# Lain-Iwakuro/Plonky2-Demo

Measured on AMD Instinct MI355X. Metric: proofs/sec for m=64 matmul circuit (full prove(), PoseidonGoldilocksConfig, standard_recursion_config), higher is better.
Workload: dtype u64 (Goldilocks, 64-bit modular integer)

## Files before the change

plonky2_demo_amd/csrc/gl64_gfx950.cuh:

```cuda
#pragma once
#include "gl64.cuh"

#if defined(__HIP_DEVICE_COMPILE__)
typedef uint32_t glx_u32x2 __attribute__((ext_vector_type(2)));
__device__ __forceinline__ gl_t glx_mk64(uint32_t lo, uint32_t hi) { glx_u32x2 v = {lo, hi}; return __builtin_bit_cast(gl_t, v); }
__device__ __forceinline__ gl_t glx_add_eps_if(gl_t z, uint32_t bit) {
    gl_t r;
    asm("v_mad_u64_u32 %0, vcc, %1, -1, %2" : "=v"(r) : "v"(bit), "v"(z) : "vcc");
    return r;
}


template <bool CANON>
__device__ __forceinline__ void glx_mul3(gl_t aA, gl_t bA, gl_t aB, gl_t bB, gl_t aC, gl_t bC, gl_t& rA, gl_t& rB, gl_t& rC) {
    typedef uint32_t u32;
    gl_t p00A, midA, p11A, p00B, midB, p11B, p00C, midC, p11C;
    uint64_t cmA, cmB, cmC;
    asm("v_mad_u64_u32 %[p00A], vcc, %[a0A], %[b0A], 0\n\t"
        "v_mad_u64_u32 %[p00B], vcc, %[a0B], %[b0B], 0\n\t"
        "v_mad_u64_u32 %[p00C], vcc, %[a0C], %[b0C], 0\n\t"
        "v_mad_u64_u32 %[midA], vcc, %[a0A], %[b1A], 0\n\t"
        "v_mad_u64_u32 %[midB], vcc, %[a0B], %[b1B], 0\n\t"
        "v_mad_u64_u32 %[midC], vcc, %[a0C], %[b1C], 0\n\t"
        "v_mad_u64_u32 %[p11A], vcc, %[a1A], %[b1A], 0\n\t"
// ... 279 lines not shown
        : [zA] "=&v"(zA), [cA] "=&s"(cA), [zB] "=&v"(zB), [cB] "=&s"(cB), [zC] "=&v"(zC), [cC] "=&s"(cC), [eA] "=&v"(eA), [eB] "=&v"(eB), [eC] "=&v"(eC)
        : [tA] "v"(topA), [loA] "v"(loA), [tB] "v"(topB), [loB] "v"(loB), [tC] "v"(topC), [loC] "v"(loC));
    rA = glx_add_eps_if(zA, eA); rB = glx_add_eps_if(zB, eB); rC = glx_add_eps_if(zC, eC);
    const uint64_t nA = whA | sA, nB = whB | sB, nC = whC | sC;
    if (__builtin_expect((wlA | wlB | wlC | nA | nB | nC) != 0, 0)) {
        u32 pA, pB, pC, mA, mB, mC;
        asm("v_cndmask_b32_e64 %[pA], 0, -1, %[wlA]\n\t"
            "v_cndmask_b32_e64 %[pB], 0, -1, %[wlB]\n\t"
            "v_cndmask_b32_e64 %[pC], 0, -1, %[wlC]\n\t"
            "v_cndmask_b32_e64 %[mA], 0, 1, %[nA]\n\t"
            "v_cndmask_b32_e64 %[mB], 0, 1, %[nB]\n\t"
            "v_cndmask_b32_e64 %[mC], 0, 1, %[nC]"
            : [pA] "=&v"(pA), [pB] "=&v"(pB), [pC] "=&v"(pC), [mA] "=&v"(mA), [mB] "=&v"(mB), [mC] "=&v"(mC)
            : [wlA] "s"(wlA), [wlB] "s"(wlB), [wlC] "s"(wlC), [nA] "s"(nA), [nB] "s"(nB), [nC] "s"(nC));
        rA = gl_sub(gl_add(rA, (gl_t)pA), (gl_t)mA); rB = gl_sub(gl_add(rB, (gl_t)pB), (gl_t)mB); rC = gl_sub(gl_add(rC, (gl_t)pC), (gl_t)mC);
    }
}

__device__ __forceinline__ gl_t glx_canon(gl_t x) { return glx_add_eps_if(x, (x >= GL_P) ? 1u : 0u); }
__device__ __forceinline__ gl_t glx_add_cc(gl_t a, gl_t b) {
    const gl_t s = a + b;
    return glx_add_eps_if(s, ((s < a) | (s >= GL_P)) ? 1u : 0u);
}
__device__ __forceinline__ gl_t glx_sub_cc(gl_t a, gl_t b) {
#ifdef GLX_C_BUTTERFLY
    const gl_t d = a - b;
    return d - ((a < b) ? GL_EPS : 0);
#endif
    uint32_t r0, r1, e;
    asm("v_sub_co_u32 %[r0], vcc, %[a0], %[b0]\n\t"
        "s_nop 1\n\t"
        "v_subb_co_u32 %[r1], vcc, %[a1], %[b1], vcc\n\t"
        "s_nop 1\n\t"
        "v_cndmask_b32_e64 %[e], 0, -1, vcc\n\t"
        "v_sub_co_u32 %[r0], vcc, %[r0], %[e]\n\t"
        "s_nop 1\n\t"
        "v_subbrev_co_u32 %[r1], vcc, 0, %[r1], vcc"
        : [r0] "=&v"(r0), [r1] "=&v"(r1), [e] "=&v"(e)
        : [a0] "v"((uint32_t)a), [a1] "v"((uint32_t)(a >> 32)), [b0] "v"((uint32_t)b), [b1] "v"((uint32_t)(b >> 32))
        : "vcc");
    return glx_mk64(r0, r1);
}
__device__ __forceinline__ void glx_sub_cc4(const gl_t (&a)[4], const gl_t (&b)[4], gl_t (&r)[4]) {
    typedef uint32_t u32;
    u32 r0A, r1A, r0B, r1B, r0C, r1C, r0D, r1D, eA, eB, eC, eD;
    uint64_t sB, sC, sD;
// ... 127 lines not shown
            : [t0] "v"((u32)term), [t1] "v"((u32)(term >> 32)),
              [wA0] "s"((u32)wA), [wA1] "s"((u32)(wA >> 32)), [wB0] "s"((u32)wB), [wB1] "s"((u32)(wB >> 32))
            : "vcc");
    }
    __device__ __forceinline__ gl_t sum(int b) const {
        gl_t r = glx_add_cc(glx_canon(a0[b]), glx_shl_c<32>(glx_canon(a1[b])));
        r = glx_add_cc(r, glx_shl_c<64>(glx_canon(a2[b])));
        r = glx_add_cc(r, glx_shl_c<64>((gl_t)k0[b]));
        r = glx_sub_cc(r, (gl_t)k1[b]);
        return glx_sub_cc(r, glx_shl_c<32>((gl_t)k2[b]));
    }
};
#elif defined(__HIPCC__)
template <bool CANON>
__device__ void glx_mul3(gl_t aA, gl_t bA, gl_t aB, gl_t bB, gl_t aC, gl_t bC, gl_t& rA, gl_t& rB, gl_t& rC);
template <bool CANON>
__device__ gl_t glx_mul(gl_t a, gl_t b);
__device__ gl_t glx_reduce96(gl_t lo, uint32_t top);
__device__ gl_t glx_mad_k(uint32_t x, uint32_t c, uint64_t k);
__device__ gl_t glx_mac_c(gl_t acc, uint32_t x, uint32_t c);
__device__ gl_t glx_canon(gl_t x);
__device__ gl_t glx_add_eps_if(gl_t z, uint32_t bit);
__device__ gl_t glx_add_cc(gl_t a, gl_t b);
__device__ gl_t glx_sub_cc(gl_t a, gl_t b);
__device__ void glx_sub_cc4(const gl_t (&a)[4], const gl_t (&b)[4], gl_t (&r)[4]);
template <int E>
__device__ gl_t glx_shl_c(gl_t x);
__device__ gl_t glx_acc_reduce(gl_t al, gl_t ah);
__device__ void glx_acc_reduce3(gl_t alA, gl_t ahA, gl_t alB, gl_t ahB, gl_t alC, gl_t ahC, gl_t& rA, gl_t& rB, gl_t& rC);
__device__ gl_t glx_mac_co(gl_t acc, uint32_t x, uint32_t c, uint64_t& carry);
__device__ void glx_acc_reduce3w(gl_t alA, gl_t ahA, uint64_t wlA, uint64_t whA, gl_t alB, gl_t ahB, uint64_t wlB, uint64_t whB,
                                 gl_t alC, gl_t ahC, uint64_t wlC, uint64_t whC, gl_t& rA, gl_t& rB, gl_t& rC);
struct GlxWideAcc2 {
    gl_t a0[2], a1[2], a2[2];
    uint32_t k0[2], k1[2], k2[2];
    __device__ void clear();
    __device__ void mac(gl_t term, gl_t wA, gl_t wB);
    __device__ gl_t sum(int b) const;
};
#endif
```

plonky2_demo_amd/csrc/merkle.hip:

```cpp
#include "context.hpp"
#include "poseidon.cuh"
#include "keccak.cuh"
#include "host_circuit.hpp"
#include <cstring>
#include <memory>

struct gl_merkle {
    gl_ctx* ctx = nullptr;
    GlMerkle tree;
    gl_t* leaves = nullptr;
    size_t num_leaves = 0, leaf_len = 0;
};

#define GL_COOP_MAX_NODES_DEFAULT 8192u
#define GL_COOP_MAX_NODES_THROUGHPUT 1024u
static uint32_t gl_coop_max_nodes() {
    static const long env = [] { const char* e = getenv("GL_COOP_MAX_NODES"); return e ? (long)strtoul(e, nullptr, 10) : -1L; }();
    if (env >= 0) return (uint32_t)env;
    return gl_proofs_in_flight.load(std::memory_order_relaxed) > 2 ? GL_COOP_MAX_NODES_THROUGHPUT : GL_COOP_MAX_NODES_DEFAULT;
}

__device__ __forceinline__ uint32_t d_bitrev(uint32_t x, uint32_t bits) { return bits ? (__brev(x) >> (32 - bits)) : 0; }

template <int WPE>
__global__ __launch_bounds__(256, WPE) void k_merkle_leaves(const gl_t* __restrict__ base, const uint64_t* __restrict__ offsets,
                                                       uint32_t leaf_len, uint32_t lg_leaves, gl_t* __restrict__ digests) {
    const uint32_t n = 1u << lg_leaves, gid = blockIdx.x * blockDim.x + threadIdx.x, r = gid < n ? gid : n - 1;
    gl_t s[12];
#pragma unroll
    for (int i = 0; i < 12; i++) s[i] = 0;
    if (leaf_len <= 4) {
        for (uint32_t e = 0; e < leaf_len; e++) s[e] = gl_canon(base[offsets[e] + r]);
    } else {
        for (uint32_t e0 = 0; e0 < leaf_len; e0 += 8) {
            const uint32_t c = leaf_len - e0 < 8 ? leaf_len - e0 : 8;
#pragma unroll
            for (int i = 0; i < 8; i++)
                if ((uint32_t)i < c) s[i] = base[offsets[e0 + i] + r];
            psd_permute_layer<PSD_LAYER_HASH>(s);
        }
    }
    if (gid >= n) return;
    const uint32_t j = d_bitrev(r, lg_leaves);
    ulonglong2* out = reinterpret_cast<ulonglong2*>(digests + 4ull * j);
    out[0] = make_ulonglong2(gl_canon(s[0]), gl_canon(s[1]));
    out[1] = make_ulonglong2(gl_canon(s[2]), gl_canon(s[3]));
}

__global__ __launch_bounds__(256, 5) void k_merkle_level(const gl_t* __restrict__ child, gl_t* __restrict__ parent, uint32_t count,
                                                         int prio ) {
    gl_raise_prio(prio);
    const uint32_t gid = blockIdx.x * blockDim.x + threadIdx.x, i = gid < count ? gid : count - 1;
    const ulonglong2* in = reinterpret_cast<const ulonglong2*>(child + 8ull * i);
    ulonglong2 a = in[0], b = in[1], c = in[2], d = in[3];
    gl_t s[12] = {a.x, a.y, b.x, b.y, c.x, c.y, d.x, d.y, 0, 0, 0, 0};
    psd_permute_layer<PSD_LAYER_HASH>(s);
    if (gid >= count) return;
    ulonglong2* out = reinterpret_cast<ulonglong2*>(parent + 4ull * i);
    out[0] = make_ulonglong2(gl_canon(s[0]), gl_canon(s[1]));
    out[1] = make_ulonglong2(gl_canon(s[2]), gl_canon(s[3]));
}

__global__ __launch_bounds__(256) void k_merkle_level_coop(const gl_t* __restrict__ child, gl_t* __restrict__ parent, uint32_t count) {
    const uint32_t gid = blockIdx.x * blockDim.x + threadIdx.x, node = gid >> 4;
    const int l = (int)(gid & 15);
    if (node >= count) return;
    gl_t s = l < 8 ? child[8ull * node + l] : 0;
    s = psd_coop_permute(s, l);
    if (l < 4) parent[4ull * node + l] = gl_canon(s);
}
__global__ __launch_bounds__(256) void k_merkle_leaves_coop(const gl_t* __restrict__ base, const uint64_t* __restrict__ offsets,
                                                            uint32_t leaf_len, uint32_t lg_leaves, gl_t* __restrict__ digests) {
    const uint32_t gid = blockIdx.x * blockDim.x + threadIdx.x, r = gid >> 4;
    const int l = (int)(gid & 15);
    if (r >= (1u << lg_leaves)) return;
    gl_t s = 0;
    if (leaf_len <= 4) {
        if ((uint32_t)l < leaf_len) s = gl_canon(base[offsets[l] + r]);
    } else {
// ... 31 lines not shown
    gl_t s[12];
#pragma unroll
    for (int k = 0; k < 12; k++) s[k] = states[12 * i + k];
    psd_permute_layer<LAYER>(s);
    if (gid >= count) return;
#pragma unroll
    for (int k = 0; k < 12; k++) states[12 * i + k] = CANON ? gl_canon(s[k]) : s[k];
}

__global__ __launch_bounds__(64, 5) void k_hash_rows(const gl_t* rows, size_t count, uint32_t len, gl_t* out) {
    const size_t gid = (size_t)blockIdx.x * blockDim.x + threadIdx.x, r = gid < count ? gid : count - 1;
    gl_t s[12];
#pragma unroll
    for (int i = 0; i < 12; i++) s[i] = 0;
    const gl_t* row = rows + r * len;
    if (len <= 4) {
        for (uint32_t e = 0; e < len; e++) s[e] = gl_canon(row[e]);
    } else {
        for (uint32_t e0 = 0; e0 < len; e0 += 8) {
            const uint32_t c = len - e0 < 8 ? len - e0 : 8;
#pragma unroll
            for (int i = 0; i < 8; i++)
                if ((uint32_t)i < c) s[i] = row[e0 + i];
            psd_permute_layer<PSD_LAYER_HASH>(s);
        }
    }
    if (gid >= count) return;
    for (int i = 0; i < 4; i++) out[4 * r + i] = gl_canon(s[i]);
}

__global__ __launch_bounds__(256) void k_kck_leaves(const gl_t* __restrict__ base, const uint64_t* __restrict__ offsets, uint32_t leaf_len,
                                                    uint32_t lg_leaves, gl_t* __restrict__ digests) {
    const uint32_t r = blockIdx.x * blockDim.x + threadIdx.x;
    if (r >= (1u << lg_leaves)) return;
    uint64_t out[4] = {0, 0, 0, 0};
    if (leaf_len * 8 <= KCK_HASH_BYTES) {
        for (uint32_t e = 0; e < leaf_len; e++) out[e] = gl_canon(base[offsets[e] + r]);
    } else {
        kck_state s;
        kck_absorb_leaf(s, leaf_len, [&](uint32_t e) { return base[offsets[e] + r]; });
        kck_digest25(s, out);
    }
    ulonglong2* o = reinterpret_cast<ulonglong2*>(digests + 4ull * d_bitrev(r, lg_leaves));
    o[0] = make_ulonglong2(out[0], out[1]);
    o[1] = make_ulonglong2(out[2], out[3]);
}
__device__ __forceinline__ void kck_node(const gl_t* __restrict__ child, gl_t* __restrict__ parent, uint32_t i) {
// ... 227 lines not shown
```

plonky2_demo_amd/csrc/poseidon.cuh:

```cuda
#pragma once
#include <stdlib.h>
#include "gl64.cuh"
#include "gl64_gfx950.cuh"
#include "poseidon_constants.h"

#if defined(__HIPCC__)
#define POSEIDON_TABLE(name, n) static __constant__ const uint64_t d_##name[n]
#define POSEIDON_TABLE32(name, n) static __constant__ const uint32_t d_##name[n]
#include "poseidon_constants.inc"
#undef POSEIDON_TABLE
#undef POSEIDON_TABLE32
#endif

#if defined(__HIP_DEVICE_COMPILE__)
#define PSD_TAB(name) d_##name
#else
#define PSD_TAB(name) name
#endif

GL_HD gl_t psd_sbox(gl_t x) {
#if defined(__HIP_DEVICE_COMPILE__)
    const gl_t x2 = glx_mul<false>(x, x), x4 = glx_mul<false>(x2, x2), x3 = glx_mul<false>(x, x2);
    return glx_mul<false>(x3, x4);
#else
// ... 76 lines not shown
        for (int i = 0; i < 12; i++) s[i] = t[i];
    }
    for (int r = 0; r < POSEIDON_PARTIAL_ROUNDS; r++) {
        const gl_t s0 = gl_add_c(psd_sbox(s[0]), POSEIDON_PARTIAL_RC[r]);
        PsdHostDot d;
        psd_host_dot_term(d, s0, 17 + 8);
        for (int i = 1; i < 12; i++) psd_host_dot_term(d, s[i], POSEIDON_PARTIAL_ROW[r * 11 + i - 1]);
        for (int i = 1; i < 12; i++) s[i] = gl_mul_add(s[i], s0, POSEIDON_PARTIAL_COL[r * 11 + i - 1]);
        s[0] = psd_host_dot_reduce(d);
    }
}

GL_HD gl_t psd_acc_reduce(gl_t al, gl_t ah) {
#if defined(__HIP_DEVICE_COMPILE__)
    return glx_acc_reduce(al, ah);
#else
    const uint32_t al_hi = (uint32_t)(al >> 32), ah_lo = (uint32_t)ah;
    const uint32_t mid = al_hi + ah_lo;
    const uint32_t top = (uint32_t)(ah >> 32) + (mid < ah_lo ? 1u : 0u);
    return gl_reduce96(((gl_t)mid << 32) | (uint32_t)al, top);
#endif
}

template <bool WITH_RC>
GL_HD void psd_mds_then_constants(gl_t (&s)[12], const gl_t* __restrict__ rc) {
    uint32_t k16 = 16, k2 = 2, k8 = 8;
#if defined(__HIP_DEVICE_COMPILE__)
    asm volatile("" : "+s"(k16), "+s"(k2), "+s"(k8));
#endif
    const uint32_t circ[12] = {17, 15, 41, k16, k2, 28, 13, 13, 39, 18, 34, 20};
    uint32_t lo[12], hi[12];
#pragma unroll
    for (int i = 0; i < 12; i++) { lo[i] = (uint32_t)s[i]; hi[i] = (uint32_t)(s[i] >> 32); }
#if defined(__HIP_DEVICE_COMPILE__)
#pragma unroll
    for (int r0 = 0; r0 < 12; r0 += 3) {
        gl_t al[3], ah[3];
#pragma unroll
        for (int k = 0; k < 3; k++) {
            const int r = r0 + k;
            if (WITH_RC) { const gl_t c = rc[r]; al[k] = glx_mad_k(lo[r], 17u, (uint64_t)(uint32_t)c); ah[k] = glx_mad_k(hi[r], 17u, c >> 32); }
            else { al[k] = (gl_t)lo[r] * 17u; ah[k] = (gl_t)hi[r] * 17u; }
#pragma unroll
            for (int i = 1; i < 12; i++) {
                al[k] += (gl_t)lo[(i + r) % 12] * circ[i];
                ah[k] += (gl_t)hi[(i + r) % 12] * circ[i];
            }
            if (r == 0) { al[k] += (gl_t)lo[0] * k8; ah[k] += (gl_t)hi[0] * k8; }
        }
        glx_acc_reduce3(al[0], ah[0], al[1], ah[1], al[2], ah[2], s[r0], s[r0 + 1], s[r0 + 2]);
    }
#else
#pragma unroll
    for (int r = 0; r < 12; r++) {
        gl_t al = 0, ah = 0;
        if (WITH_RC) { const gl_t c = rc[r]; al = (uint32_t)c; ah = c >> 32; }
#pragma unroll
        for (int i = 0; i < 12; i++) {
            al += (gl_t)lo[(i + r) % 12] * circ[i];
// ... 9 lines not shown
#define PSD_MDS_MFMA 1
#endif
#ifndef PSD_GROUP4
#define PSD_GROUP4 1
#endif
enum { PSD_LAYER_VALU = 0, PSD_LAYER_MFMA = 1, PSD_LAYER_HASH = PSD_MDS_MFMA ? PSD_LAYER_MFMA : PSD_LAYER_VALU };
#if defined(__HIPCC__)
typedef int psd_i32x4 __attribute__((ext_vector_type(4)));
typedef int psd_i32x16 __attribute__((ext_vector_type(16)));
struct PsdMfmaA { psd_i32x4 blk[4]; };
#endif
#if defined(__HIP_DEVICE_COMPILE__)
__device__ __forceinline__ PsdMfmaA psd_mfma_a() {
    const uint32_t lane = __builtin_amdgcn_mbcnt_hi(~0u, __builtin_amdgcn_mbcnt_lo(~0u, 0u)), r = lane & 31;
    const bool mine = ((r >> 2) & 1) == (lane >> 5);
    const uint32_t o8 = 8 * (r >> 3), t8 = 8 * (r & 3);
    PsdMfmaA A;
#pragma unroll
    for (int d = 0; d < 4; d++)
#pragma unroll
        for (int q = 0; q < 4; q++) A.blk[d][q] = mine ? (int)(((d_POSEIDON_MDS_I8A[4 * d + q] >> o8) & 0xFFu) << t8) : 0;
    return A;
}
__device__ __forceinline__ void psd_mds_mfma(gl_t (&s)[12], const gl_t* __restrict__ kk, const PsdMfmaA& A) {
    psd_i32x4 bl[3], bh[3];
#pragma unroll
    for (int kb = 0; kb < 3; kb++)
#pragma unroll
        for (int q = 0; q < 4; q++) {
            bl[kb][q] = (int)((uint32_t)s[4 * kb + q] ^ 0x80808080u);
            bh[kb][q] = (int)((uint32_t)(s[4 * kb + q] >> 32) ^ 0x80808080u);
        }
    int32_t one = 1, m8 = 1 << 8, m16 = 1 << 16, m24 = 1 << 24;
    asm volatile("" : "+v"(one), "+s"(m8), "+s"(m16), "+s"(m24));
    gl_t acc[2][12];
#pragma unroll
    for (int rb = 0; rb < 3; rb++) {
#pragma unroll
        for (int hf = 0; hf < 2; hf++) {
            __builtin_amdgcn_sched_barrier(0);
            psd_i32x16 d = {};
#pragma unroll
            for (int kb = 0; kb < 3; kb++)
                d = __builtin_amdgcn_mfma_i32_32x32x32_i8((rb == 0 && kb == 0) ? A.blk[3] : A.blk[(kb - rb + 3) % 3], hf ? bh[kb] : bl[kb], d, 0, 0, 0);
#pragma unroll
            for (int o = 0; o < 4; o++) {
                const int i = 4 * rb + o;
                int64_t x = (int64_t)d[4 * o] * one + (int64_t)kk[2 * i + hf];
                x += (int64_t)d[4 * o + 1] * m8;
                x += (int64_t)d[4 * o + 2] * m16;
                x += (int64_t)d[4 * o + 3] * m24;
                acc[hf][i] = (gl_t)x;
            }
        }
#pragma unroll
        for (int r0 = 3 * rb; r0 < 4 * rb + 2; r0 += 3)
            glx_acc_reduce3(acc[0][r0], acc[1][r0], acc[0][r0 + 1], acc[1][r0 + 1], acc[0][r0 + 2], acc[1][r0 + 2], s[r0], s[r0 + 1], s[r0 + 2]);
    }
    __builtin_amdgcn_sched_barrier(0);
}
#endif

GL_HD constexpr uint32_t psd_mds_entry(int r, int c) {
    constexpr uint32_t circ[12] = {17, 15, 41, 16, 2, 28, 13, 13, 39, 18, 34, 20};
    return circ[(c - r + 12) % 12] + ((r == 0 && c == 0) ? 8u : 0u);
}
GL_HD void psd_sbox_all(gl_t (&s)[12]) {
#if defined(__HIP_DEVICE_COMPILE__)
#pragma unroll
    for (int k = 0; k < 12; k += 3) {
        gl_t a2, b2, c2, a4, b4, c4, a3, b3, c3;
        glx_mul3<false>(s[k], s[k], s[k + 1], s[k + 1], s[k + 2], s[k + 2], a2, b2, c2);
        glx_mul3<false>(a2, a2, b2, b2, c2, c2, a4, b4, c4);
        glx_mul3<false>(s[k], a2, s[k + 1], b2, s[k + 2], c2, a3, b3, c3);
        glx_mul3<false>(a3, a4, b3, b4, c3, c4, s[k], s[k + 1], s[k + 2]);
    }
#else
    for (int i = 0; i < 12; i++) s[i] = psd_sbox(s[i]);
#endif
}
#if defined(__HIPCC__)
template <bool SUBST>
__device__ __forceinline__ void psd_partial_group_k(gl_t (&s)[12], const gl_t* __restrict__ K, const gl_t* in, gl_t* a) {
    uint32_t z = 0;
#if defined(__HIP_DEVICE_COMPILE__)
    asm volatile("" : "+s"(z));
#endif
    const uint32_t* __restrict__ R2 = d_POSEIDON_G3_R2 + z;
    const uint32_t* __restrict__ V1 = d_POSEIDON_G3_V1 + z;
    a[0] = s[0];
    s[0] = psd_sbox(SUBST ? in[0] : s[0]);
    uint32_t lo[12], hi[12];
#pragma unroll
// ... 63 lines not shown
    const gl_t d3 = gl_sub(psd_sbox(a3), a3);
    const uint32_t d3l = (uint32_t)d3, d3h = (uint32_t)(d3 >> 32);
    const uint32_t* __restrict__ M4 = d_POSEIDON_G4_M4 + z;
#pragma unroll
    for (int l0 = 0; l0 < 12; l0 += 3) {
        gl_t xl[3], xh[3];
        uint64_t wl[3], wh[3];
#pragma unroll
        for (int k = 0; k < 3; k++) {
            const int l = l0 + k;
            xl[k] = glx_mad_k(d3l, psd_mds_entry(l, 0), (uint64_t)(uint32_t)K[3 + l]); xh[k] = glx_mad_k(d3h, psd_mds_entry(l, 0), K[3 + l] >> 32);
#pragma unroll
            for (int i = 1; i < 12; i++) { const uint32_t c = M4[12 * l + i]; xl[k] += (gl_t)lo[i] * c; xh[k] += (gl_t)hi[i] * c; }
            { const uint32_t c = V3[l]; xl[k] += (gl_t)d1l * c; xh[k] += (gl_t)d1h * c; }
            { const uint32_t c = V2[l]; xl[k] += (gl_t)d2l * c; xh[k] += (gl_t)d2h * c; }
            { const uint32_t c = M4[12 * l]; xl[k] = glx_mac_co(xl[k], lo[0], c, wl[k]); xh[k] = glx_mac_co(xh[k], hi[0], c, wh[k]); }
        }
        glx_acc_reduce3w(xl[0], xh[0], wl[0], wh[0], xl[1], xh[1], wl[1], wh[1], xl[2], xh[2], wl[2], wh[2], s[l0], s[l0 + 1], s[l0 + 2]);
    }
}
#endif

#if defined(__HIP_DEVICE_COMPILE__)
template <int LAYER, bool WITH_RC>
__device__ __forceinline__ void psd_mds_layer(gl_t (&s)[12], int n, const PsdMfmaA& A) {
    if constexpr (LAYER == PSD_LAYER_MFMA) psd_mds_mfma(s, d_POSEIDON_MDS_K + 24 * (WITH_RC ? n : 8 + POSEIDON_PARTIAL_ROUNDS), A);
    else psd_mds_then_constants<WITH_RC>(s, WITH_RC ? d_POSEIDON_RC + 12 * n : nullptr);
}
template <int LAYER>
__device__ __forceinline__ void psd_permute_layer(gl_t (&s)[12]) {
    const gl_t* __restrict__ rc = d_POSEIDON_RC;
    PsdMfmaA A;
    if constexpr (LAYER == PSD_LAYER_MFMA) A = psd_mfma_a();
#pragma unroll
    for (int i = 0; i < 12; i++) s[i] = gl_add_c(s[i], rc[i]);
#if PSD_GROUP4
#pragma unroll 1
    for (int r = 0; r < 4; r++) { psd_sbox_all(s); if (r < 3) psd_mds_layer<LAYER, true>(s, r + 1, A); }
#pragma unroll 1
    for (int g = 0; g < POSEIDON_G4_GROUPS; g++) psd_partial_group4(s, d_POSEIDON_G4_K + 15 * g, g != 0);
    { gl_t a[3]; psd_partial_group_k<false>(s, d_POSEIDON_G4_K + 15 * POSEIDON_G4_GROUPS, nullptr, a); }
#else
#pragma unroll 1
    for (int r = 0; r < 4; r++) { psd_sbox_all(s); psd_mds_layer<LAYER, true>(s, r + 1, A); }
#pragma unroll 1
    for (int g = 0; g < POSEIDON_PARTIAL_GROUPS; g++) { gl_t a[3]; psd_partial_group<false>(s, g, nullptr, a); }
#pragma unroll 1
    for (int r = 4 + 3 * POSEIDON_PARTIAL_GROUPS; r < 4 + POSEIDON_PARTIAL_ROUNDS; r++) { s[0] = psd_sbox(s[0]); psd_mds_layer<LAYER, true>(s, r + 1, A); }
#endif
#pragma unroll 1
    for (int r = 4 + POSEIDON_PARTIAL_ROUNDS; r < 7 + POSEIDON_PARTIAL_ROUNDS; r++) { psd_sbox_all(s); psd_mds_layer<LAYER, true>(s, r + 1, A); }
    psd_sbox_all(s);
    psd_mds_layer<LAYER, false>(s, 0, A);
}
GL_HD void psd_permute(gl_t (&s)[12]) { psd_permute_layer<PSD_LAYER_VALU>(s); }
#else
#if defined(__HIPCC__)
template <int LAYER>
__device__ void psd_permute_layer(gl_t (&s)[12]);
#endif
GL_HD void psd_permute(gl_t (&s)[12]) {
    for (int r = 0; r < 4; r++) psd_full_round(s, r);
    psd_partial_rounds(s);
    for (int r = 0; r < 4; r++) psd_full_round(s, 4 + POSEIDON_PARTIAL_ROUNDS + r);
}
#endif

#if defined(__HIPCC__)
__device__ __forceinline__ gl_t psd_coop_permute(gl_t s, const int l) {
    const uint32_t circ[12] = {17, 15, 41, 16, 2, 28, 13, 13, 39, 18, 34, 20};
    const gl_t* __restrict__ rc = d_POSEIDON_RC;
    const int lc = l < 12 ? l : 0;
    const int lane = (int)(threadIdx.x & 63), row = lane & ~15;
    s = gl_add_c(s, rc[lc]);
#pragma unroll 1
    for (int r = 0; r < 8 + POSEIDON_PARTIAL_ROUNDS; r++) {
        const bool full = r < 4 || r >= 4 + POSEIDON_PARTIAL_ROUNDS;
        if (full || l == 0) s = psd_sbox(s);
        const uint32_t lo = (uint32_t)s, hi = (uint32_t)(s >> 32);
        gl_t al = 0, ah = 0;
        if (r + 1 < 8 + POSEIDON_PARTIAL_ROUNDS) { const gl_t c = rc[12 * (r + 1) + lc]; al = (uint32_t)c; ah = c >> 32; }
        al = glx_mac_c(al, lo, 17u); ah = glx_mac_c(ah, hi, 17u);
// ... 25 lines not shown
```

plonky2_demo_amd/csrc/poseidon_constants.inc:

```
POSEIDON_TABLE(POSEIDON_RC, 360) = {
    0xb585f766f2144405ULL, 0x7746a55f43921ad7ULL, 0xb2fb0d31cee799b4ULL, 0x0f6760a4803427d7ULL,
    0xe10d666650f4e012ULL, 0x8cae14cb07d09bf1ULL, 0xd438539c95f63e9fULL, 0xef781c7ce35b4c3dULL,
    0xcdc4a239b0c44426ULL, 0x277fa208bf337bffULL, 0xe17653a29da578a1ULL, 0xc54302f225db2c76ULL,
    0x86287821f722c881ULL, 0x59cd1a8a41c18e55ULL, 0xc3b919ad495dc574ULL, 0xa484c4c5ef6a0781ULL,
    0x308bbd23dc5416ccULL, 0x6e4a40c18f30c09cULL, 0x9a2eedb70d8f8cfaULL, 0xe360c6e0ae486f38ULL,
    0xd5c7718fbfc647fbULL, 0xc35eae071903ff0bULL, 0x849c2656969c4be7ULL, 0xc0572c8c08cbbbadULL,
    0xe9fa634a21de0082ULL, 0xf56f6d48959a600dULL, 0xf7d713e806391165ULL, 0x8297132b32825dafULL,
    0xad6805e0e30b2c8aULL, 0xac51d9f5fcf8535eULL, 0x502ad7dc18c2ad87ULL, 0x57a1550c110b3041ULL,
    0x66bbd30e6ce0e583ULL, 0x0da2abef589d644eULL, 0xf061274fdb150d61ULL, 0x28b8ec3ae9c29633ULL,
    0x92a756e67e2b9413ULL, 0x70e741ebfee96586ULL, 0x019d5ee2af82ec1cULL, 0x6f6f2ed772466352ULL,
    0x7cf416cfe7e14ca1ULL, 0x61df517b86a46439ULL, 0x85dc499b11d77b75ULL, 0x4b959b48b9c10733ULL,
    0xe8be3e5da8043e57ULL, 0xf5c0bc1de6da8699ULL, 0x40b12cbf09ef74bfULL, 0xa637093ecb2ad631ULL,
    0x3cc3f892184df408ULL, 0x2e479dc157bf31bbULL, 0x6f49de07a6234346ULL, 0x213ce7bede378d7bULL,
    0x5b0431345d4dea83ULL, 0xa2de45780344d6a1ULL, 0x7103aaf94a7bf308ULL, 0x5326fc0d97279301ULL,
    0xa9ceb74fec024747ULL, 0x27f8ec88bb21b1a3ULL, 0xfceb4fda1ded0893ULL, 0xfac6ff1346a41675ULL,
    0x7131aa45268d7d8cULL, 0x9351036095630f9fULL, 0xad535b24afc26bfbULL, 0x4627f5c6993e44beULL,
    0x645cf794b8f1cc58ULL, 0x241c70ed0af61617ULL, 0xacb8e076647905f1ULL, 0x3737e9db4c4f474dULL,
    0xe7ea5e33e75fffb6ULL, 0x90dee49fc9bfc23aULL, 0xd1b1edf76bc09c92ULL, 0x0b65481ba645c602ULL,
    0x99ad1aab0814283bULL, 0x438a7c91d416ca4dULL, 0xb60de3bcc5ea751cULL, 0xc99cab6aef6f58bcULL,
    0x69a5ed92a72ee4ffULL, 0x5e7b329c1ed4ad71ULL, 0x5fc0ac0800144885ULL, 0x32db829239774ecaULL,
    0x0ade699c5830f310ULL, 0x7cc5583b10415f21ULL, 0x85df9ed2e166d64fULL, 0x6604df4fee32bcb1ULL,
    0xeb84f608da56ef48ULL, 0xda608834c40e603dULL, 0x8f97fe408061f183ULL, 0xa93f485c96f37b89ULL,
    0x6704e8ee8f18d563ULL, 0xcee3e9ac1e072119ULL, 0x510d0e65e2b470c1ULL, 0xf6323f486b9038f0ULL,
    0x0b508cdeffa5ceefULL, 0xf2417089e4fb3cbdULL, 0x60e75c2890d15730ULL, 0xa6217d8bf660f29cULL,
// ... 502 lines not shown
    0x0000008171d7d0cdULL, 0x000000809d075265ULL, 0x000000815e03ac1cULL, 0x00000080ba174e73ULL,
    0x0000008118b2a4bdULL, 0x000000810f003a02ULL, 0x0000008083a5ddd4ULL, 0x000000813a8e6c71ULL,
    0x0000008096a97c5bULL, 0x000000811f1d3d78ULL, 0x00000081176e56a5ULL, 0x000000815b68e459ULL,
    0x0000008132225378ULL, 0x000000815f3e8853ULL, 0x00000080cd81c343ULL, 0x000000812512a9d2ULL,
    0x000000855f14e21cULL, 0x00000085006a3dffULL, 0x0000008142c52a30ULL, 0x000000812449deaeULL,
    0x00000081755f8544ULL, 0x0000008082b13ca8ULL, 0x000000814061c8c6ULL, 0x00000080c1b642beULL,
    0x00000080c40abc72ULL, 0x0000008096f040ccULL, 0x000000810b68befaULL, 0x00000080b7e3359aULL,
    0x000000810991c750ULL, 0x0000008169130a4cULL, 0x000000812514dee5ULL, 0x00000080aac48b51ULL,
    0x00000080fe1a7f83ULL, 0x00000081014f7d2bULL, 0x0000008166a0562aULL, 0x000000813c18f9c6ULL,
    0x0000008104a6d034ULL, 0x00000080eefd0f1aULL, 0x000000809c3f5dc8ULL, 0x0000008096cc32deULL,
    0x00000084d1e0e93bULL, 0x000000857845b3e5ULL, 0x000000816e17f1e2ULL, 0x00000080c13a6922ULL,
    0x000000813efb9840ULL, 0x00000080d59fdb0fULL, 0x00000081454b9811ULL, 0x00000080a583aaa7ULL,
    0x00000080cb96c346ULL, 0x000000812b6db407ULL, 0x000000817a4a481dULL, 0x00000081107e16bbULL,
    0x00000080d9b7885cULL, 0x00000080f17d11ebULL, 0x00000080e011d440ULL, 0x00000080fff9de2aULL,
    0x00000080d4f753cbULL, 0x00000080c5c459dfULL, 0x0000008080d0490dULL, 0x0000008171f3573eULL,
    0x000000813d489238ULL, 0x00000081605244feULL, 0x000000810065d8fcULL, 0x000000813d0e7b62ULL,
    0x0000008484848400ULL, 0x0000008484848400ULL, 0x0000008080808000ULL, 0x0000008080808000ULL,
    0x0000008080808000ULL, 0x0000008080808000ULL, 0x0000008080808000ULL, 0x0000008080808000ULL,
    0x0000008080808000ULL, 0x0000008080808000ULL, 0x0000008080808000ULL, 0x0000008080808000ULL,
    0x0000008080808000ULL, 0x0000008080808000ULL, 0x0000008080808000ULL, 0x0000008080808000ULL,
    0x0000008080808000ULL, 0x0000008080808000ULL, 0x0000008080808000ULL, 0x0000008080808000ULL,
    0x0000008080808000ULL, 0x0000008080808000ULL, 0x0000008080808000ULL, 0x0000008080808000ULL,
};
```

plonky2_demo_amd/csrc/prover_kernels.cuh:

```cuda
#pragma once
#include "gl64.cuh"
#include "poseidon.cuh"
#include "keccak.cuh"
#include "gates.hpp"
#include "../../include/plonky2_mi355x.h"

#define GLP_MAX_ROUTED 80
#define GLP_CHUNKS 10

struct GlPermParams {
    const gl_t* wires;
    const gl_t* sigmas;
    const gl_t* xpow_lo; const gl_t* xpow_hi;
    gl_t k_is[GLP_MAX_ROUTED];
    gl_t betas[2], gammas[2];
    uint32_t n;
    uint32_t k_is_powers_of_7;
    gl_t* chunk_prod;
    gl_t* row_prod;
};

__device__ __forceinline__ gl_t glp_pow2level(const gl_t* lo, const gl_t* hi, uint32_t e) {
    return gl_mul(lo[e & 2047], hi[e >> 11]);
}
// ... 222 lines not shown
    const gl_t* zs = p.zs + i;
    GlAlphaAcc terms; terms.start(p.alpha_pows);
    gl_t tot0 = 0, tot1 = 0;
    if constexpr (!POSEIDON_PART) {
    const gl_t x = glx_canon(glp_pow2level(p.xpow_lo, p.xpow_hi, i));
    const uint32_t i_next = (i + p.next_step) & (uint32_t)(N - 1);
    const gl_t l0 = p.l0_coset[i];
    gl_t bx0, bx1, lz0, lz1, bxk0, bxk1, unused;
    glx_mul3<true>(p.betas[0], x, p.betas[1], x, l0, glx_sub_cc(zs[0], 1), bx0, bx1, lz0);
    terms.add(0, lz0);
    glx_mul3<true>(bx0, p.k_is[0], bx1, p.k_is[0], l0, glx_sub_cc(zs[N], 1), bxk0, bxk1, lz1);
    terms.add(1, lz1);
    {
        const gl_t beta0 = p.betas[0], beta1 = p.betas[1], gamma0 = p.gammas[0], gamma1 = p.gammas[1];
        gl_t prev0 = zs[0], prev1 = zs[N];
#pragma unroll 1
        for (int c = 0; c < GLP_CHUNKS; c++) {
            gl_t n0 = 1, d0 = 1, n1 = 1, d1 = 1;
#pragma unroll
            for (int q = 0; q < 8; q++) {
                const int j = c * 8 + q;
                const gl_t wv = w[(size_t)j * N], sg = cs[(size_t)(p.num_constants + j) * N];
                if (!p.k_is_powers_of_7) { const gl_t k = p.k_is[j]; glx_mul3<true>(bx0, k, bx1, k, 0, 0, bxk0, bxk1, unused); }
                const gl_t f0 = glx_add_cc(glx_add_cc(wv, bxk0), gamma0), f1 = glx_add_cc(glx_add_cc(wv, bxk1), gamma1);
                gl_t sb0, sb1;
                glx_mul3<true>(sg, beta0, sg, beta1, n0, f0, sb0, sb1, n0);
                const gl_t g0 = glx_add_cc(glx_add_cc(wv, sb0), gamma0), g1 = glx_add_cc(glx_add_cc(wv, sb1), gamma1);
                glx_mul3<true>(d0, g0, n1, f1, d1, g1, d0, n1, d1);
                if (p.k_is_powers_of_7) {
                    bxk0 = glx_sub_cc(glx_shl_c<3>(bxk0), bxk0); bxk1 = glx_sub_cc(glx_shl_c<3>(bxk1), bxk1);
                }
            }
            const gl_t next0 = (c == GLP_CHUNKS - 1) ? p.zs[i_next] : zs[(size_t)(2 + c) * N];
            const gl_t next1 = (c == GLP_CHUNKS - 1) ? p.zs[N + i_next] : zs[(size_t)(2 + (GLP_CHUNKS - 1) + c) * N];
            gl_t pn0, nd0, pn1, nd1;
            glx_mul3<true>(prev0, n0, next0, d0, prev1, n1, pn0, nd0, pn1);
            nd1 = glx_mul<true>(next1, d1);
            terms.add(2 + c, glx_sub_cc(pn0, nd0));
            terms.add(2 + GLP_CHUNKS + c, glx_sub_cc(pn1, nd1));
            prev0 = next0; prev1 = next1;
        }
    }
    tot0 = terms.sum(0); tot1 = terms.sum(1);
    }
    const uint32_t T0 = p.gate_term0;
    const gl_t* gc = cs + (size_t)(p.num_selectors + p.num_lookup_selectors) * N;
#pragma unroll 1
    for (uint32_t g = 0; g < p.num_gates; g++) {
        if ((p.gate_types[g] == glhost::G_POSEIDON) != POSEIDON_PART) continue;
        const gl_t sel = cs[(size_t)p.gate_sel[g] * N];
        gl_t filter = 1;
// ... 586 lines not shown
    for (int t = 0; t < B; t++) b[t] = gl2_make(carries[2 * ((size_t)t * nseg + s)], carries[2 * ((size_t)t * nseg + s) + 1]);
    for (uint32_t k = hi; k > lo; k--) {
        gl2_t q = gl2_make(0, 0);
#pragma unroll
        for (int t = 0; t < B; t++) {
            q = gl2_add(q, gl2_mul(b[t], gl2_make(pt.scale[t][0], pt.scale[t][1])));
            b[t] = gl2_add(gl2_mul(b[t], gl2_make(pt.z[t][0], pt.z[t][1])), gl2_make(F[(size_t)(2 * t) * n + k - 1], F[(size_t)(2 * t + 1) * n + k - 1]));
        }
        qa[k - 1] = gl_canon(q.a); qb[k - 1] = gl_canon(q.b);
    }
}

__global__ __launch_bounds__(256) void k_fri_fold(const gl_t* ia, const gl_t* ib, uint32_t n_out, uint32_t arity, gl_t ba, gl_t bb, gl_t* oa, gl_t* ob, int prio) {
    gl_raise_prio(prio);
    const uint32_t k = blockIdx.x * blockDim.x + threadIdx.x;
    if (k >= n_out) return;
    const gl2_t beta = gl2_make(ba, bb);
    gl2_t acc = gl2_make(0, 0);
    for (uint32_t i = arity; i-- > 0;) acc = gl2_add(gl2_mul(acc, beta), gl2_make(ia[(size_t)arity * k + i], ib[(size_t)arity * k + i]));
    oa[k] = gl_canon(acc.a); ob[k] = gl_canon(acc.b);
}

struct GlPowParams { gl_t state[12]; uint32_t pos, min_leading_zeros; uint64_t base, count; unsigned long long* result; int prio ; };
__global__ __launch_bounds__(256, 5) void k_pow_grind(GlPowParams p) {
    gl_raise_prio(p.prio);
    const uint64_t idx = (uint64_t)blockIdx.x * blockDim.x + threadIdx.x;
    const uint64_t cand = p.base + idx;
    gl_t s[12];
#pragma unroll
    for (int i = 0; i < 12; i++) s[i] = p.state[i];
#pragma unroll
    for (int i = 0; i < 8; i++) if ((uint32_t)i == p.pos) s[i] = cand;
    psd_permute_layer<PSD_LAYER_HASH>(s);
    const gl_t r = gl_canon(s[7]);
    const uint32_t lz = r ? (uint32_t)__clzll((long long)r) : 64u;
    if (idx < p.count && lz >= p.min_leading_zeros) atomicMin(p.result, (unsigned long long)cand);
}
__global__ __launch_bounds__(256) void k_kck_pow_grind(GlPowParams p) {
    const uint64_t idx = (uint64_t)blockIdx.x * blockDim.x + threadIdx.x;
    if (idx >= p.count) return;
    const uint64_t cand = p.base + idx;
    gl_t s[12], e[8];
#pragma unroll
    for (int i = 0; i < 12; i++) s[i] = p.state[i];
#pragma unroll
    for (int i = 0; i < 8; i++) if ((uint32_t)i == p.pos) s[i] = cand;
    kck_onion<8>(s, e);
    const gl_t r = e[7];
    const uint32_t lz = r ? (uint32_t)__clzll((long long)r) : 64u;
    if (lz >= p.min_leading_zeros) atomicMin(p.result, (unsigned long long)cand);
}

enum { GLG_ROWS = 0, GLG_PATHS = 1, GLG_FRI_LEAVES = 2 };
#define GLG_MAX_PIECES 32
struct GlGatherPiece {
    const gl_t* src; const gl_t* src2;
    const uint64_t* level_off;
    uint64_t stride, out_off;
    uint32_t kind, a, b, count, idx_off, pad_;
};
__global__ __launch_bounds__(256) void k_gather_pieces(const GlGatherPiece* __restrict__ pieces, uint32_t npieces, const uint32_t* __restrict__ idx,
                                                       gl_t* __restrict__ out, int prio) {
// ... 27 lines not shown
```

Before: 370.1.

## Prune unused Poseidon outputs, precompute zero-capacity sbox, early-exit pow grind

Adds a KEEP mask to the final MDS layer so permutations compute only the output lanes that are later read: digest lanes for Merkle nodes, capacity lanes for sponge absorbs that overwrite the rate, and lane 7 for proof-of-work. The first-round sbox on an all-zero capacity is replaced by precomputed constants. Pow grind waves exit early when a lower candidate has already been found. The permutation-argument kernel uses non-canonical multiplies and a one-carry add to drop canonicalisations. These changes add template variants and risk correctness if the lane masks or non-canonical bounds are wrong.

```diff
diff --git a/plonky2_demo_amd/csrc/gl64_gfx950.cuh b/plonky2_demo_amd/csrc/gl64_gfx950.cuh
--- a/plonky2_demo_amd/csrc/gl64_gfx950.cuh
+++ b/plonky2_demo_amd/csrc/gl64_gfx950.cuh
@@ -325,6 +325,10 @@
     const gl_t s = a + b;
     return glx_add_eps_if(s, ((s < a) | (s >= GL_P)) ? 1u : 0u);
 }
+__device__ __forceinline__ gl_t glx_add_1c(gl_t a, gl_t b) {
+    const gl_t s = a + b;
+    return glx_add_eps_if(s, (s < a) ? 1u : 0u);
+}
 __device__ __forceinline__ gl_t glx_sub_cc(gl_t a, gl_t b) {
 #ifdef GLX_C_BUTTERFLY
     const gl_t d = a - b;
@@ -498,6 +502,7 @@
 __device__ gl_t glx_canon(gl_t x);
 __device__ gl_t glx_add_eps_if(gl_t z, uint32_t bit);
 __device__ gl_t glx_add_cc(gl_t a, gl_t b);
+__device__ gl_t glx_add_1c(gl_t a, gl_t b);
 __device__ gl_t glx_sub_cc(gl_t a, gl_t b);
 __device__ void glx_sub_cc4(const gl_t (&a)[4], const gl_t (&b)[4], gl_t (&r)[4]);
 template <int E>
diff --git a/plonky2_demo_amd/csrc/merkle.hip b/plonky2_demo_amd/csrc/merkle.hip
--- a/plonky2_demo_amd/csrc/merkle.hip
+++ b/plonky2_demo_amd/csrc/merkle.hip
@@ -37,7 +37,10 @@
 #pragma unroll
             for (int i = 0; i < 8; i++)
                 if ((uint32_t)i < c) s[i] = base[offsets[e0 + i] + r];
-            psd_permute_layer<PSD_LAYER_HASH>(s);
+            if constexpr (WPE == 5) {
+                const uint32_t left = leaf_len - e0 - c;
+                psd_sponge_permute<PSD_LAYER_HASH>(s, e0 == 0, left < 8 ? left : 8);
+            } else psd_permute_layer<PSD_LAYER_HASH>(s);
         }
     }
     if (gid >= n) return;
@@ -54,7 +57,7 @@
     const ulonglong2* in = reinterpret_cast<const ulonglong2*>(child + 8ull * i);
     ulonglong2 a = in[0], b = in[1], c = in[2], d = in[3];
     gl_t s[12] = {a.x, a.y, b.x, b.y, c.x, c.y, d.x, d.y, 0, 0, 0, 0};
-    psd_permute_layer<PSD_LAYER_HASH>(s);
+    psd_permute_layer<PSD_LAYER_HASH, PSD_KEEP_DIGEST, true>(s);
     if (gid >= count) return;
     ulonglong2* out = reinterpret_cast<ulonglong2*>(parent + 4ull * i);
     out[0] = make_ulonglong2(gl_canon(s[0]), gl_canon(s[1]));
@@ -132,7 +135,8 @@
 #pragma unroll
             for (int i = 0; i < 8; i++)
                 if ((uint32_t)i < c) s[i] = row[e0 + i];
-            psd_permute_layer<PSD_LAYER_HASH>(s);
+            const uint32_t left = len - e0 - c;
+            psd_sponge_permute<PSD_LAYER_HASH>(s, e0 == 0, left < 8 ? left : 8);
         }
     }
     if (gid >= count) return;
diff --git a/plonky2_demo_amd/csrc/poseidon.cuh b/plonky2_demo_amd/csrc/poseidon.cuh
--- a/plonky2_demo_amd/csrc/poseidon.cuh
+++ b/plonky2_demo_amd/csrc/poseidon.cuh
@@ -122,7 +122,8 @@
 #endif
 }
 
-template <bool WITH_RC>
+enum : uint32_t { PSD_KEEP_ALL = 0xFFFu, PSD_KEEP_DIGEST = 0x00Fu, PSD_KEEP_CAPACITY = 0xF00u };
+template <bool WITH_RC, uint32_t KEEP = PSD_KEEP_ALL>
 GL_HD void psd_mds_then_constants(gl_t (&s)[12], const gl_t* __restrict__ rc) {
     uint32_t k16 = 16, k2 = 2, k8 = 8;
 #if defined(__HIP_DEVICE_COMPILE__)
@@ -135,6 +136,7 @@
 #if defined(__HIP_DEVICE_COMPILE__)
 #pragma unroll
     for (int r0 = 0; r0 < 12; r0 += 3) {
+        if (!((KEEP >> r0) & 7u)) continue;
         gl_t al[3], ah[3];
 #pragma unroll
         for (int k = 0; k < 3; k++) {
@@ -190,6 +192,7 @@
         for (int q = 0; q < 4; q++) A.blk[d][q] = mine ? (int)(((d_POSEIDON_MDS_I8A[4 * d + q] >> o8) & 0xFFu) << t8) : 0;
     return A;
 }
+template <uint32_t KEEP>
 __device__ __forceinline__ void psd_mds_mfma(gl_t (&s)[12], const gl_t* __restrict__ kk, const PsdMfmaA& A) {
     psd_i32x4 bl[3], bh[3];
 #pragma unroll
@@ -199,6 +202,9 @@
             bl[kb][q] = (int)((uint32_t)s[4 * kb + q] ^ 0x80808080u);
             bh[kb][q] = (int)((uint32_t)(s[4 * kb + q] >> 32) ^ 0x80808080u);
         }
+#pragma unroll
+    for (int i = 0; i < 12; i++)
+        if (!((KEEP >> i) & 1u)) asm("" : "=v"(s[i]));
     int32_t one = 1, m8 = 1 << 8, m16 = 1 << 16, m24 = 1 << 24;
     asm volatile("" : "+v"(one), "+s"(m8), "+s"(m16), "+s"(m24));
     gl_t acc[2][12];
@@ -206,6 +212,7 @@
     for (int rb = 0; rb < 3; rb++) {
 #pragma unroll
         for (int hf = 0; hf < 2; hf++) {
+            if (!((KEEP >> (4 * rb)) & 0xFu)) continue;
             __builtin_amdgcn_sched_barrier(0);
             psd_i32x16 d = {};
 #pragma unroll
@@ -214,6 +221,7 @@
 #pragma unroll
             for (int o = 0; o < 4; o++) {
                 const int i = 4 * rb + o;
+                if (!((KEEP >> i) & 1u)) continue;
                 int64_t x = (int64_t)d[4 * o] * one + (int64_t)kk[2 * i + hf];
                 x += (int64_t)d[4 * o + 1] * m8;
                 x += (int64_t)d[4 * o + 2] * m16;
@@ -222,8 +230,15 @@
             }
         }
 #pragma unroll
-        for (int r0 = 3 * rb; r0 < 4 * rb + 2; r0 += 3)
-            glx_acc_reduce3(acc[0][r0], acc[1][r0], acc[0][r0 + 1], acc[1][r0 + 1], acc[0][r0 + 2], acc[1][r0 + 2], s[r0], s[r0 + 1], s[r0 + 2]);
+        for (int r0 = 3 * rb; r0 < 4 * rb + 2; r0 += 3) {
+            if (((KEEP >> r0) & 7u) == 7u)
+                glx_acc_reduce3(acc[0][r0], acc[1][r0], acc[0][r0 + 1], acc[1][r0 + 1], acc[0][r0 + 2], acc[1][r0 + 2], s[r0], s[r0 + 1], s[r0 + 2]);
+            else {
+#pragma unroll
+                for (int r = r0; r < r0 + 3; r++)
+                    if ((KEEP >> r) & 1u) s[r] = glx_acc_reduce(acc[0][r], acc[1][r]);
+            }
+        }
     }
     __builtin_amdgcn_sched_barrier(0);
 }
@@ -233,10 +248,15 @@
     constexpr uint32_t circ[12] = {17, 15, 41, 16, 2, 28, 13, 13, 39, 18, 34, 20};
     return circ[(c - r + 12) % 12] + ((r == 0 && c == 0) ? 8u : 0u);
 }
-GL_HD void psd_sbox_all(gl_t (&s)[12]) {
+GL_HD void psd_sbox_all(gl_t (&s)[12], bool cap0 = false) {
 #if defined(__HIP_DEVICE_COMPILE__)
 #pragma unroll
     for (int k = 0; k < 12; k += 3) {
+        if (k == 9 && cap0) {
+#pragma unroll
+            for (int i = 9; i < 12; i++) s[i] = d_POSEIDON_CAP0_SBOX[i - 8];
+            continue;
+        }
         gl_t a2, b2, c2, a4, b4, c4, a3, b3, c3;
         glx_mul3<false>(s[k], s[k], s[k + 1], s[k + 1], s[k + 2], s[k + 2], a2, b2, c2);
         glx_mul3<false>(a2, a2, b2, b2, c2, c2, a4, b4, c4);
@@ -346,42 +366,57 @@
 #endif
 
 #if defined(__HIP_DEVICE_COMPILE__)
-template <int LAYER, bool WITH_RC>
+template <int LAYER, bool WITH_RC, uint32_t KEEP = PSD_KEEP_ALL>
 __device__ __forceinline__ void psd_mds_layer(gl_t (&s)[12], int n, const PsdMfmaA& A) {
-    if constexpr (LAYER == PSD_LAYER_MFMA) psd_mds_mfma(s, d_POSEIDON_MDS_K + 24 * (WITH_RC ? n : 8 + POSEIDON_PARTIAL_ROUNDS), A);
-    else psd_mds_then_constants<WITH_RC>(s, WITH_RC ? d_POSEIDON_RC + 12 * n : nullptr);
+    if constexpr (LAYER == PSD_LAYER_MFMA) psd_mds_mfma<KEEP>(s, d_POSEIDON_MDS_K + 24 * (WITH_RC ? n : 8 + POSEIDON_PARTIAL_ROUNDS), A);
+    else psd_mds_then_constants<WITH_RC, KEEP>(s, WITH_RC ? d_POSEIDON_RC + 12 * n : nullptr);
 }
 template <int LAYER>
+__device__ __forceinline__ void psd_permute_rounds(gl_t (&s)[12], const PsdMfmaA& A, bool cap0) {
+    const gl_t* __restrict__ rc = d_POSEIDON_RC;
+#pragma unroll
+    for (int i = 0; i < 12; i++) s[i] = gl_add_c(s[i], rc[i]);
+#if PSD_GROUP4
+#pragma unroll 1
+    for (int r = 0; r < 4; r++) { psd_sbox_all(s, cap0 && r == 0); if (r < 3) psd_mds_layer<LAYER, true>(s, r + 1, A); }
+#pragma unroll 1
+    for (int g = 0; g < POSEIDON_G4_GROUPS; g++) psd_partial_group4(s, d_POSEIDON_G4_K + 15 * g, g != 0);
+    { gl_t a[3]; psd_partial_group_k<false>(s, d_POSEIDON_G4_K + 15 * POSEIDON_G4_GROUPS, nullptr, a); }
+#else
+#pragma unroll 1
+    for (int r = 0; r < 4; r++) { psd_sbox_all(s, cap0 && r == 0); psd_mds_layer<LAYER, true>(s, r + 1, A); }
+#pragma unroll 1
+    for (int g = 0; g < POSEIDON_PARTIAL_GROUPS; g++) { gl_t a[3]; psd_partial_group<false>(s, g, nullptr, a); }
+#pragma unroll 1
+    for (int r = 4 + 3 * POSEIDON_PARTIAL_GROUPS; r < 4 + POSEIDON_PARTIAL_ROUNDS; r++) { s[0] = psd_sbox(s[0]); psd_mds_layer<LAYER, true>(s, r + 1, A); }
+#endif
+#pragma unroll 1
+    for (int r = 4 + POSEIDON_PARTIAL_ROUNDS; r < 7 + POSEIDON_PARTIAL_ROUNDS; r++) { psd_sbox_all(s); psd_mds_layer<LAYER, true>(s, r + 1, A); }
+    psd_sbox_all(s);
+}
+template <int LAYER, uint32_t KEEP = PSD_KEEP_ALL, bool CAP0 = false>
 __device__ __forceinline__ void psd_permute_layer(gl_t (&s)[12]) {
-    const gl_t* __restrict__ rc = d_POSEIDON_RC;
     PsdMfmaA A;
     if constexpr (LAYER == PSD_LAYER_MFMA) A = psd_mfma_a();
-#pragma unroll
-    for (int i = 0; i < 12; i++) s[i] = gl_add_c(s[i], rc[i]);
-#if PSD_GROUP4
-#pragma unroll 1
-    for (int r = 0; r < 4; r++) { psd_sbox_all(s); if (r < 3) psd_mds_layer<LAYER, true>(s, r + 1, A); }
-#pragma unroll 1
-    for (int g = 0; g < POSEIDON_G4_GROUPS; g++) psd_partial_group4(s, d_POSEIDON_G4_K + 15 * g, g != 0);
-    { gl_t a[3]; psd_partial_group_k<false>(s, d_POSEIDON_G4_K + 15 * POSEIDON_G4_GROUPS, nullptr, a); }
-#else
-#pragma unroll 1
-    for (int r = 0; r < 4; r++) { psd_sbox_all(s); psd_mds_layer<LAYER, true>(s, r + 1, A); }
-#pragma unroll 1
-    for (int g = 0; g < POSEIDON_PARTIAL_GROUPS; g++) { gl_t a[3]; psd_partial_group<false>(s, g, nullptr, a); }
-#pragma unroll 1
-    for (int r = 4 + 3 * POSEIDON_PARTIAL_GROUPS; r < 4 + POSEIDON_PARTIAL_ROUNDS; r++) { s[0] = psd_sbox(s[0]); psd_mds_layer<LAYER, true>(s, r + 1, A); }
-#endif
-#pragma unroll 1
-    for (int r = 4 + POSEIDON_PARTIAL_ROUNDS; r < 7 + POSEIDON_PARTIAL_ROUNDS; r++) { psd_sbox_all(s); psd_mds_layer<LAYER, true>(s, r + 1, A); }
-    psd_sbox_all(s);
-    psd_mds_layer<LAYER, false>(s, 0, A);
+    psd_permute_rounds<LAYER>(s, A, CAP0);
+    psd_mds_layer<LAYER, false, KEEP>(s, 0, A);
+}
+template <int LAYER>
+__device__ __forceinline__ void psd_sponge_permute(gl_t (&s)[12], bool first, uint32_t next) {
+    PsdMfmaA A;
+    if constexpr (LAYER == PSD_LAYER_MFMA) A = psd_mfma_a();
+    psd_permute_rounds<LAYER>(s, A, first);
+    if (next == 8) psd_mds_layer<LAYER, false, PSD_KEEP_CAPACITY>(s, 0, A);
+    else if (next == 0) psd_mds_layer<LAYER, false, PSD_KEEP_DIGEST>(s, 0, A);
+    else psd_mds_layer<LAYER, false>(s, 0, A);
 }
 GL_HD void psd_permute(gl_t (&s)[12]) { psd_permute_layer<PSD_LAYER_VALU>(s); }
 #else
 #if defined(__HIPCC__)
+template <int LAYER, uint32_t KEEP = PSD_KEEP_ALL, bool CAP0 = false>
+__device__ void psd_permute_layer(gl_t (&s)[12]);
 template <int LAYER>
-__device__ void psd_permute_layer(gl_t (&s)[12]);
+__device__ void psd_sponge_permute(gl_t (&s)[12], bool first, uint32_t next);
 #endif
 GL_HD void psd_permute(gl_t (&s)[12]) {
     for (int r = 0; r < 4; r++) psd_full_round(s, r);
diff --git a/plonky2_demo_amd/csrc/poseidon_constants.inc b/plonky2_demo_amd/csrc/poseidon_constants.inc
--- a/plonky2_demo_amd/csrc/poseidon_constants.inc
+++ b/plonky2_demo_amd/csrc/poseidon_constants.inc
@@ -548,3 +548,6 @@
     0x0000008080808000ULL, 0x0000008080808000ULL, 0x0000008080808000ULL, 0x0000008080808000ULL,
     0x0000008080808000ULL, 0x0000008080808000ULL, 0x0000008080808000ULL, 0x0000008080808000ULL,
 };
+POSEIDON_TABLE(POSEIDON_CAP0_SBOX, 4) = {
+    0xc70fa963a6d76d43ULL, 0x8046358185c6e230ULL, 0x6e54c050fb2a6ae5ULL, 0xb1742ab4a8c81453ULL,
+};
diff --git a/plonky2_demo_amd/csrc/prover_kernels.cuh b/plonky2_demo_amd/csrc/prover_kernels.cuh
--- a/plonky2_demo_amd/csrc/prover_kernels.cuh
+++ b/plonky2_demo_amd/csrc/prover_kernels.cuh
@@ -268,11 +268,12 @@
                 const int j = c * 8 + q;
                 const gl_t wv = w[(size_t)j * N], sg = cs[(size_t)(p.num_constants + j) * N];
                 if (!p.k_is_powers_of_7) { const gl_t k = p.k_is[j]; glx_mul3<true>(bx0, k, bx1, k, 0, 0, bxk0, bxk1, unused); }
-                const gl_t f0 = glx_add_cc(glx_add_cc(wv, bxk0), gamma0), f1 = glx_add_cc(glx_add_cc(wv, bxk1), gamma1);
+                const gl_t wg0 = glx_add_cc(wv, gamma0), wg1 = glx_add_cc(wv, gamma1);
+                const gl_t f0 = glx_add_cc(wg0, bxk0), f1 = glx_add_cc(wg1, bxk1);
                 gl_t sb0, sb1;
-                glx_mul3<true>(sg, beta0, sg, beta1, n0, f0, sb0, sb1, n0);
-                const gl_t g0 = glx_add_cc(glx_add_cc(wv, sb0), gamma0), g1 = glx_add_cc(glx_add_cc(wv, sb1), gamma1);
-                glx_mul3<true>(d0, g0, n1, f1, d1, g1, d0, n1, d1);
+                glx_mul3<false>(sg, beta0, sg, beta1, n0, f0, sb0, sb1, n0);
+                const gl_t g0 = glx_add_1c(sb0, wg0), g1 = glx_add_1c(sb1, wg1);
+                glx_mul3<false>(d0, g0, n1, f1, d1, g1, d0, n1, d1);
                 if (p.k_is_powers_of_7) {
                     bxk0 = glx_sub_cc(glx_shl_c<3>(bxk0), bxk0); bxk1 = glx_sub_cc(glx_shl_c<3>(bxk1), bxk1);
                 }
@@ -905,22 +906,30 @@
 }
 
 struct GlPowParams { gl_t state[12]; uint32_t pos, min_leading_zeros; uint64_t base, count; unsigned long long* result; int prio ; };
+__device__ __forceinline__ bool gl_pow_wave_is_beaten(const unsigned long long* result, uint64_t cand) {
+    const unsigned long long seen = __hip_atomic_load(result, __ATOMIC_RELAXED, __HIP_MEMORY_SCOPE_AGENT);
+    const uint64_t lowest = (uint64_t)__builtin_amdgcn_readfirstlane((uint32_t)cand) | ((uint64_t)__builtin_amdgcn_readfirstlane((uint32_t)(cand >> 32)) << 32);
+    const uint64_t best = (uint64_t)__builtin_amdgcn_readfirstlane((uint32_t)seen) | ((uint64_t)__builtin_amdgcn_readfirstlane((uint32_t)(seen >> 32)) << 32);
+    return lowest > best;
+}
 __global__ __launch_bounds__(256, 5) void k_pow_grind(GlPowParams p) {
     gl_raise_prio(p.prio);
     const uint64_t idx = (uint64_t)blockIdx.x * blockDim.x + threadIdx.x;
     const uint64_t cand = p.base + idx;
+    if (gl_pow_wave_is_beaten(p.result, cand)) return;
     gl_t s[12];
 #pragma unroll
     for (int i = 0; i < 12; i++) s[i] = p.state[i];
 #pragma unroll
     for (int i = 0; i < 8; i++) if ((uint32_t)i == p.pos) s[i] = cand;
-    psd_permute_layer<PSD_LAYER_HASH>(s);
+    psd_permute_layer<PSD_LAYER_HASH, 1u << 7>(s);
     const gl_t r = gl_canon(s[7]);
     const uint32_t lz = r ? (uint32_t)__clzll((long long)r) : 64u;
     if (idx < p.count && lz >= p.min_leading_zeros) atomicMin(p.result, (unsigned long long)cand);
 }
 __global__ __launch_bounds__(256) void k_kck_pow_grind(GlPowParams p) {
     const uint64_t idx = (uint64_t)blockIdx.x * blockDim.x + threadIdx.x;
+    if (gl_pow_wave_is_beaten(p.result, p.base + idx)) return;
     if (idx >= p.count) return;
     const uint64_t cand = p.base + idx;
     gl_t s[12], e[8];
```

Result: faster. 374.4, median of 6 (+1.2%).
